# Bioinfo-Tools/PANGEA-plus

Measured on AMD Instinct MI355X. Metric: classified reads/sec (+ HBM GB/s fraction), 150 bp vs 1 Gbp db, 1/2/4/8 GPU, higher is better.
Workload: dtype u64 (2-bit packed bases, integer scores)

## Files before the change

pangea-plus_amd/csrc/classify.hip:

```cpp
#include <algorithm>
#include <chrono>

#include "bitops.hpp"
#include "consensus_core.hpp"
#include "engine.hpp"
#include "read_order.hpp"

#include <rocprim/device/device_radix_sort.hpp>

namespace pgx {

struct Diag {
	const uint64_t *rw, *ra;
	const uint64_t *dbw, *dba;
	int64_t dstart;
	int lo, hi;
};

template <bool AMB> __device__ __forceinline__ uint64_t mmw(const Diag &D, int w)
{
	int b0 = 32 * w;
	if (b0 + 32 <= D.lo || b0 >= D.hi)
		return kEven;
	uint64_t x = D.rw[w] ^ window64(D.dbw, D.dstart + b0);
// ... 1473 lines not shown
		const uint32_t k32 = kept ? dec_str_key32(rmv) : 0u;
		uint32_t kmax = k32;
#pragma unroll
		for (int m = 1; m < G; m <<= 1)
			kmax = max(kmax, (uint32_t)__shfl_xor(kmax, m));
		const bool elig = kept && k32 == kmax;
		if (PGX_SORT_DBG(cv) == 6) {
			if (__ballot(elig && slow && !present) && li == 0)
				recs[r].hit = 0;
			continue;
		}
		if (PGX_SORT_DBG(cv) != 4) {
			const uint32_t key2 = elig ? ((sim << 6) | (63u - rank)) + 1u : 0u;
			uint32_t top = key2;
#pragma unroll
			for (int m = 1; m < G; m <<= 1)
				top = max(top, (uint32_t)__shfl_xor(top, m));
			if (elig && key2 == top && present && !slow) {
				recs[r].hit = (int32_t)(o + rank);
				recs[r].matches = (int32_t)rmv;
			}
		}
		if (odd_mask) {
			const bool any_huge = __ballot(kept && (rmv >= 100000000u || ntok >= 100000000u || sim >= (1u << 25))) != 0ull;
			lds_fence();
			if (any_huge) {
				if (kept) {
					sw->b.rm[slot0 + rank] = rmv;
					sw->b.sim[slot0 + rank] = sim;
					sw->b.krm[slot0 + rank] = dec_str_key(rmv);
					sw->b.kcnt[slot0 + rank] = dec_str_key(ntok);
				}
				lds_fence();
				if (li == 0 && n && slow && present) {
					ArgmaxState am;
					am.cursim = r == 0 ? cv.simrank_undef : cv.simrank_zero;
					for (uint32_t k = 0; k < n; k++)
						am.step_keys((int32_t)(o + k), sw->b.rm[slot0 + k], sw->b.krm[slot0 + k], sw->b.kcnt[slot0 + k],
							     sw->b.sim[slot0 + k]);
					recs[r].hit = am.win;
					recs[r].matches = (int32_t)am.maxrm;
				}
			} else {
				const uint32_t c32 = dec_str_key32(ntok);
				if (kept) {
					sw->c.kcnt[slot0 + rank] = c32;
					sw->c.sim_e[slot0 + rank] = sim | (elig ? 0x80000000u : 0u);
					sw->c.krm[slot0 + rank] = k32;
					sw->c.rm[slot0 + rank] = rmv;
				}
				lds_fence();
				if (n && slow && present) {
					const bool top_is_max = (sw->c.sim_e[slot0] >> 31) != 0u;
					const uint32_t init_sim = r == 0 ? cv.simrank_undef : cv.simrank_zero;
					if (top_is_max) {
						uint32_t nx = kNoRead;
						for (uint32_t t = 0; t < n; t++) {
							const uint32_t a = sw->c.kcnt[slot0 + t], b2 = sw->c.sim_e[slot0 + t];
							const bool cand = kept && t > rank && (b2 >> 31) && (a > c32 || (b2 & 0x7FFFFFFFu) > sim);
							nx = (cand && nx == kNoRead) ? t : nx;
						}
						if (kept)
							sw->c.nxt[slot0 + rank] = nx;
						lds_fence();
						if (li == 0) {
							uint32_t w = kNoRead;
							if (sw->c.rm[slot0] > 0u) {
								w = 0;
							} else {
								for (uint32_t t = 0; t < n && w == kNoRead; t++)
									if (sw->c.kcnt[slot0 + t] > 1u  || (sw->c.sim_e[slot0 + t] & 0x7FFFFFFFu) > init_sim)
										w = t;
							}
							if (w != kNoRead) {
								for (uint32_t nxw = sw->c.nxt[slot0 + w]; nxw != kNoRead; nxw = sw->c.nxt[slot0 + w])
									w = nxw;
								recs[r].hit = (int32_t)(o + w);
								recs[r].matches = (int32_t)sw->c.rm[slot0 + w];
							} else {
								recs[r].hit = -1;
								recs[r].matches = 0;
							}
						}
					} else if (li == 0) {
						uint32_t kr = 1u , mrm = 0, kc = 1u, cs = init_sim;
						int32_t win = -1;
						for (uint32_t k = 0; k < n; k++) {
							const uint32_t vkrm = sw->c.krm[slot0 + k], vrm = sw->c.rm[slot0 + k], vkc = sw->c.kcnt[slot0 + k],
								       vs = sw->c.sim_e[slot0 + k] & 0x7FFFFFFFu;
							if (vkrm > kr) {
								kr = vkrm;
								mrm = vrm;
								win = (int32_t)(o + k);
								cs = vs;
							}
							if ((vkc > kc || cs < vs) && vrm == mrm) {
								kc = vkc;
								win = (int32_t)(o + k);
								cs = vs;
							}
						}
						recs[r].hit = win;
						recs[r].matches = (int32_t)mrm;
					}
				}
			}
		}
		lds_fence();
	}
	if (G != 64 && lane == 0 && chunk_used < 64u && chunk_used > 0)
		for (uint32_t k = chunk_used; k < 64u; k++)
			next_list[chunk_base + k] = kNoRead;
}

__global__ void k_consensus_serial(const pgx_hit *__restrict__ hits, const uint32_t *__restrict__ off,
				   const uint32_t *__restrict__ cnt, const uint32_t *__restrict__ list, uint32_t n_list,
				   ConsView cv, pgx_consensus_rec *__restrict__ recs)
{
	uint32_t t = blockIdx.x * blockDim.x + threadIdx.x;
	if (t >= n_list)
		return;
	const uint32_t r = list ? list[t] : t;
	const uint32_t o = off[r], n = cnt[r];
	pgx_consensus_rec rec;
	rec.hit = n ? -1 : -2;
	rec.matches = 0;
	if (cv.rdp_present && !cv.rdp_present[r])
		rec.hit = -2;
	if (rec.hit == -1) {
		const uint32_t r0 = cv.rdp_off[r], r1 = cv.rdp_off[r + 1];
		ArgmaxState am;
		am.cursim = r == 0 ? cv.simrank_undef : cv.simrank_zero;
		for (uint32_t k = 0; k < n; k++) {
			const pgx_hit h = hits[o + k];
			uint32_t c;
			const uint32_t rm = hit_rank_matches(cv, (uint32_t)h.subject, r0, r1, &c);
			am.step((int32_t)(o + k), rm, c, hit_simrank(cv, h));
		}
		rec.hit = am.win;
		rec.matches = (int32_t)am.maxrm;
	}
	recs[r] = rec;
}

__global__ void k_slice_offsets(const uint32_t *__restrict__ off, const uint32_t *__restrict__ cnt, uint32_t first, uint32_t n,
				 uint32_t *__restrict__ off_out, uint32_t *__restrict__ cnt_out)
{
	const uint32_t i = blockIdx.x * blockDim.x + threadIdx.x;
	if (i <= n)
		off_out[i] = off[first + i] - off[first];
	if (i < n)
		cnt_out[i] = cnt[first + i];
}

__global__ void k_slice_hits(const pgx_hit *__restrict__ in, uint64_t base, uint64_t n_slots, uint32_t first, pgx_hit *__restrict__ out)
{
	for (uint64_t i = (uint64_t)blockIdx.x * blockDim.x + threadIdx.x; i < n_slots; i += (uint64_t)gridDim.x * blockDim.x) {
		pgx_hit h = in[base + i];
		h.read -= (int32_t)first;
		out[i] = h;
	}
}

static thread_local pgx_stage_times t_times;

static DbView db_view(const pgx_db *db)
{
	DbView v;
	v.words = db->d_words.data();
	v.amb = db->has_amb ? db->d_amb.data() : nullptr;
	v.seq_off = db->d_seq_off.data();
	v.blk_subj = db->d_blk_subj.data();
	v.blk_info = db->d_blk_info.data();
	v.post_ctx = db->d_post_ctx.data();
	v.amb_blk = db->has_amb ? db->d_amb_blk.data() : nullptr;
	v.bucket_off = db->d_bucket_off.data();
	v.postings = db->d_postings.data();
	v.n_seq = (uint32_t)db->n_seq;
	v.n_bases = db->n_bases;
	v.bits = db->index_bits;
	v.gapped = db->ungapped ? 0 : 1;
	v.deep_from = kGapDeepFrom;
#ifdef PGX_STAGE_PROBES
	v.dbg_stop = getenv("PGX_SEED_STOP") ? atoi(getenv("PGX_SEED_STOP")) : 0;
#else
	v.dbg_stop = 0;
#endif
	return v;
}

static ReadsView reads_view(const pgx_reads *rd)
{
	ReadsView v;
	v.fwd = rd->d_fwd.data();
	v.rc = rd->d_rc.data();
	v.fwd_amb = rd->has_amb ? rd->d_fwd_amb.data() : nullptr;
	v.rc_amb = rd->has_amb ? rd->d_rc_amb.data() : nullptr;
	v.len = rd->d_len.data();
	v.woff = rd->d_woff.data();
	v.n = (uint32_t)rd->n;
	v.list = nullptr;
	v.ticket = nullptr;
	v.dustwin_f = rd->has_dust ? rd->dustb.win_f.data() : nullptr;
	v.dustwin_r = rd->has_dust ? rd->dustb.win_r.data() : nullptr;
	v.dust_any = rd->has_dust ? rd->dustb.any.data() : nullptr;
	return v;
}

static ConsView cons_view(const pgx_db *db, const pgx_rdp *rdp)
{
	ConsView cv;
	memset(&cv, 0, sizeof cv);
#ifdef PGX_STAGE_PROBES
	cv.dbg = getenv("PGX_SORT_STOP") ? atoi(getenv("PGX_SORT_STOP")) : 0;
#else
	cv.dbg = 0;
#endif
	if (db && db->bound) {
		cv.subj_tok_off = db->d_subj_tok_off.data();
		cv.subj_tok = db->d_subj_tok.data();
		cv.tok_rank = db->d_tok_rank.data();
		cv.subj_pairs = db->d_subj_pairs.data();
		cv.pair_words = db->pair_words;
		cv.simrank_lut = db->d_simrank_lut.data();
		cv.simrank_len = db->d_simrank_len.data();
		cv.simrank_undef = db->simrank_undef;
		cv.simrank_zero = db->simrank_zero;
	}
	cv.np_max = db ? db->max_pairs : 15;
	cv.nr_max = rdp ? rdp->max_trip : kRdpRegs;
	if (rdp) {
		cv.rdp_off = rdp->d_off.data();
		cv.rdp_name = rdp->d_name.data();
		cv.rdp_rank = rdp->d_rank.data();
		cv.rdp_present = rdp->d_present.data();
		cv.rdp_code = rdp->d_code.data();
	}
	return cv;
}

struct StageEvents {
	static constexpr int kN = 10;
	hipEvent_t e[kN] = {};
	bool ok = false;
	int init()
	{
		if (ok)
			return 0;
		for (auto &x : e)
			PGX_HIP(hipEventCreate(&x));
		ok = true;
		return 0;
	}
	void mark(int i, hipStream_t s) { (void)hipEventRecord(e[i], s); }
	float ms(int a, int b) const
	{
		float t = 0;
		(void)hipEventElapsedTime(&t, e[a], e[b]);
		return t;
	}
};

__global__ __launch_bounds__(256) void k_merge_pieces(const pgx_hit *__restrict__ scratch, const uint32_t *__restrict__ piece_start,
						      const uint32_t *__restrict__ piece_off, const uint32_t *__restrict__ parent,
						      const uint32_t *__restrict__ qoff, uint32_t n_pieces, pgx_hit *__restrict__ hits,
						      unsigned long long hits_cap, unsigned long long scratch_cap)
{
	const uint32_t waves = gridDim.x * (blockDim.x / 64), lane = threadIdx.x & 63;
	for (uint32_t s = blockIdx.x * (blockDim.x / 64) + (threadIdx.x >> 6); s < n_pieces; s += waves) {
		const uint32_t o = piece_off[s], cnt = piece_off[s + 1] - o;
		if (cnt == 0 || (unsigned long long)o + cnt > hits_cap)
			continue;
		const uint32_t st = piece_start[s];
		if (st != kFragmented && (unsigned long long)st + cnt > scratch_cap)
			continue;
		const pgx_hit *src = st == kFragmented ? hits + o : scratch + st;
		const int32_t read = (int32_t)parent[s], shift = (int32_t)qoff[s];
		for (uint32_t i = lane; i < cnt; i += 64) {
			pgx_hit h = src[i];
			h.read = read;
			h.qstart += shift;
			h.qend += shift;
			hits[o + i] = h;
		}
	}
}

__global__ void k_piece_ranges(const uint32_t *__restrict__ piece_first, const uint32_t *__restrict__ piece_off, uint32_t n_reads,
			       uint32_t *__restrict__ read_off, uint32_t *__restrict__ read_cnt, uint32_t *__restrict__ read_start)
{
	const uint32_t r = blockIdx.x * blockDim.x + threadIdx.x;
	if (r > n_reads)
		return;
	const uint32_t o = piece_off[piece_first[r]];
	read_off[r] = o;
	if (r < n_reads) {
		read_cnt[r] = piece_off[piece_first[r + 1]] - o;
		read_start[r] = kFragmented;
	}
}

struct Workspace {
	hipStream_t stream = nullptr;
	StageEvents ev;
	DevBuf<unsigned long long> counters;
	unsigned long long *h_counters = nullptr;
	DevBuf<pgx_hit> scratch, ovf;
	DevBuf<uint8_t> scratch_key, ovf_key;
	DevBuf<uint8_t> scratch_reg;
	DevBuf<uint32_t> partial, cursor, big_list, read_start, mid_list;
	DevBuf<uint32_t> piece_cnt, piece_off, parent_start;
	DevBuf<pgx_consensus_rec> recs;
	GappedWork gapped;
	DustBufs dust;
	DevBuf<uint32_t> order_key_in, order_val_in, order_key, order_list;
	DevBuf<uint8_t> order_tmp;
	DevBuf<uint32_t> order_ticket;
	uint64_t order_n = 0;
	pgx_hits hits;
	uint64_t hit_cap_hint = 0, ovf_cap_hint = 0;
	double table_per_read_hint = 0.0;
	pgx_stage_times times;
	int device = -1;
	~Workspace()
	{
		if (h_counters)
			(void)hipHostFree(h_counters);
		if (stream)
			(void)hipStreamDestroy(stream);
	}
};
constexpr int kNCounters = 12;

static int workspace_of(pgx_db *db, Workspace **out)
{
	if (!db->work) {
		auto w = std::make_shared<Workspace>();
		PGX_HIP(hipGetDevice(&w->device));
		PGX_HIP(hipStreamCreate(&w->stream));
		PGX_HIP(hipHostMalloc((void **)&w->h_counters, (kNCounters + 3) * sizeof(unsigned long long)));
		PGX_TRY(w->ev.init());
		PGX_TRY(w->counters.alloc(kNCounters, 0, 0, true));
		db->work = w;
	}
	*out = static_cast<Workspace *>(db->work.get());
	return 0;
}

int db_stream(pgx_db *db, hipStream_t *out)
{
	Workspace *ws = nullptr;
	PGX_TRY(workspace_of(db, &ws));
	*out = ws->stream;
	return 0;
}

constexpr uint64_t kOrderMinReads = 1u << 22;
constexpr uint64_t kOrderMinDbBytes = 32ull << 20;
static bool order_wanted(const pgx_db *db, uint64_t class_reads)
{
	if (db->read_order == 1)
		return class_reads > 0;
	if (db->read_order == 2)
		return false;
	return class_reads >= kOrderMinReads && (uint64_t)db->n_bases / 4 >= kOrderMinDbBytes;
}

static int order_reads(const pgx_db *db, const DbView &dv, const ReadsView &rv, const pgx_reads *sr, Workspace &ws,
		       std::vector<int64_t> &ordered)
{
	hipStream_t st = ws.stream;
	const std::vector<pgx_reads::SearchClass> &classes = sr->classes;
	ordered.assign(classes.size(), -1);
	const int shift = read_order_shift(dv.n_bases), key_bits = read_order_key_bits(dv.n_bases);
	const uint32_t last_bin = read_order_last_bin(dv.n_bases);
	uint64_t total = 0;
	size_t tmp_bytes = 0;
	for (size_t c = 0; c < classes.size(); c++)
		if (order_wanted(db, classes[c].count)) {
			ordered[c] = (int64_t)total;
			total += classes[c].count;
			size_t bytes = 0;
			PGX_HIP(rocprim::radix_sort_pairs(nullptr, bytes, (uint32_t *)nullptr, (uint32_t *)nullptr, (uint32_t *)nullptr, (uint32_t *)nullptr,
							  (size_t)classes[c].count, 0, key_bits, st));
			tmp_bytes = std::max(tmp_bytes, bytes);
		}
	ws.order_n = total;
	if (total == 0)
		return 0;
	PGX_TRY(ws.order_key_in.ensure(total));
	PGX_TRY(ws.order_val_in.ensure(total));
	PGX_TRY(ws.order_key.ensure(total));
	PGX_TRY(ws.order_list.ensure(total));
	PGX_TRY(ws.order_tmp.ensure(tmp_bytes ? tmp_bytes : 1));
	PGX_TRY(ws.order_ticket.ensure(classes.size()));
	for (size_t c = 0; c < classes.size(); c++) {
		if (ordered[c] < 0)
			continue;
		const uint64_t o = (uint64_t)ordered[c], cn = classes[c].count;
		ReadsView cvw = rv;
		cvw.n = (uint32_t)cn;
		cvw.list = classes[c].listed ? sr->d_class_list.data() + classes[c].off : nullptr;
		hipLaunchKernelGGL(k_read_order_keys, dim3((unsigned)((cn + 255) / 256)), dim3(256), 0, st, dv, cvw, shift, last_bin, (uint32_t)c,
				   ws.order_key_in.data() + o, ws.order_val_in.data() + o);
		PGX_HIP(hipGetLastError());
		size_t bytes = ws.order_tmp.n;
		PGX_HIP(rocprim::radix_sort_pairs(ws.order_tmp.data(), bytes, ws.order_key_in.data() + o, ws.order_key.data() + o,
						  ws.order_val_in.data() + o, ws.order_list.data() + o, (size_t)cn, 0, key_bits, st));
	}
	trace_point("order_reads");
	return 0;
}

int search_pipeline(pgx_db *db, pgx_reads *rd, const pgx_rdp *rdp, pgx_hits *out, pgx_consensus_rec *d_recs)
{
	PGX_TRY(require_device());
	if (rdp && !db->bound)
		return fail(PGX_E_ARG, "consensus needs pgx_db_bind_taxonomy() first");
	if (rdp && rdp->n != rd->n)
		return fail(PGX_E_ARG, "RDP stream holds %lld reads, batch holds %lld", (long long)rdp->n, (long long)rd->n);
	std::lock_guard<std::mutex> lock(db->search_mu);
	static const bool laps_on = getenv("PGX_CALL_LAPS") != nullptr;
	const auto lap_t0 = std::chrono::steady_clock::now();
	auto lap = [&](const char *what) {
		if (laps_on)
			fprintf(stderr, "[pgx lap] %8.2f ms  %s\n", std::chrono::duration<double, std::milli>(std::chrono::steady_clock::now() - lap_t0).count(), what);
	};
	trace_point("search_pipeline: entered");
	Workspace *wsp = nullptr;
	PGX_TRY(workspace_of(db, &wsp));
	Workspace &ws = *wsp;
	hipStream_t st = ws.stream;
	pgx_stage_times &tm = ws.times;
	memset(&tm, 0, sizeof tm);
	ws.order_n = 0;
	const uint64_t n = (uint64_t)rd->n;
	out->n_reads = rd->n;
	PGX_TRY(out->d_read_cnt.ensure(n + 1));
	PGX_TRY(out->d_read_off.ensure(n + 1));
	if (n == 0) {
		out->n_hits = 0;
		t_times = tm;
		return 0;
	}
	index_check(db, "search_pipeline");
	const DbView dv = db_view(db);
	const bool split = rd->pieces && rd->pieces->n > 0;
	const pgx_reads *sr = split ? rd->pieces.get() : rd;
	const uint64_t ns = (uint64_t)sr->n;
	if (split) {
		PGX_TRY(ws.piece_cnt.ensure(ns + 1));
		PGX_TRY(ws.piece_off.ensure(ns + 1));
		PGX_TRY(ws.parent_start.ensure(n));
	}
	ReadsView rv = reads_view(sr);
	if (!db->dust)
		rv.dustwin_f = rv.dustwin_r = nullptr;
	const int grid = (int)std::min<uint64_t>((n + kWavesPerBlock - 1) / kWavesPerBlock, 256ull * 8);

	uint64_t cap = std::max<uint64_t>(std::max<uint64_t>(std::max(n, ns) * 40, 1 << 16) + 256ull * 8 * kWavesPerBlock * kChunk, ws.hit_cap_hint);
	uint64_t ovf_cap = std::max<uint64_t>(std::max<uint64_t>(std::max(n, ns) / 4, 1 << 16), ws.ovf_cap_hint);
	uint64_t table_cap = std::max<uint64_t>(std::max<uint64_t>(std::max(n, ns) * 36, 1 << 16), (uint64_t)((double)std::max(n, ns) * ws.table_per_read_hint) + 1);
	DevBuf<pgx_hit> &scratch = ws.scratch, &ovf = ws.ovf;
	DevBuf<uint32_t> &read_start = ws.read_start;
	PGX_TRY(read_start.ensure(std::max(n, ns)));
	unsigned long long *h_cnt = ws.h_counters;
	const std::vector<pgx_reads::SearchClass> &classes = sr->classes;
	bool long_reads = false;
	for (auto &c : classes)
		long_reads = long_reads || c.words == 0;
	const uint32_t n_part = (uint32_t)((ns + kScanBlock * kScanItems - 1) / (kScanBlock * kScanItems));
	PGX_TRY(ws.partial.ensure(n_part));
	PGX_TRY(ws.cursor.ensure(ns));
	PGX_TRY(ws.big_list.ensure(n));
	PGX_TRY(ws.mid_list.ensure(n + 64ull * kWavesPerBlock * 256 * 8));
	trace_point("search_pipeline: lists ready");
	const ConsView cv = cons_view(db, rdp);
	const int lds_ok = rd->max_len <= 65535 ? 1 : 0;
	uint64_t H = 0, H_ovf = 0;
	ws.ev.mark(6, st);
	const bool dust_now = db->dust && db->dust_each_search;
	if (dust_now) {
		PGX_TRY(reads_dust_again(sr, ws.dust, st));
		if (sr->has_dust) {
			rv.dustwin_f = ws.dust.win_f.data();
			rv.dustwin_r = ws.dust.win_r.data();
			rv.dust_any = ws.dust.any.data();
		}
	}
	ws.ev.mark(7, st);
	std::vector<int64_t> ordered;
	PGX_TRY(order_reads(db, dv, rv, sr, ws, ordered));
	const bool order_now = ws.order_n > 0;
	if (order_now)
		ws.ev.mark(8, st);
	for (int attempt = 0;; attempt++) {
		if (attempt > 8)
			return fail(PGX_E_LIMIT, "hit tables did not settle after %d attempts", attempt);
		PGX_TRY(scratch.ensure(cap));
		PGX_TRY(ovf.ensure(ovf_cap));
		trace_point("search_pipeline: seed tables ready");
		PGX_TRY(out->d_hits.ensure(table_cap));
		trace_point("search_pipeline: hit table ready");
		cap = scratch.n;
		ovf_cap = ovf.n;
		if (dv.gapped) {
			PGX_TRY(ws.scratch_key.ensure(cap + 16));
			PGX_TRY(ws.scratch_reg.ensure(cap + 16));
			PGX_TRY(ws.ovf_key.ensure(ovf_cap));
			PGX_HIP(hipMemsetAsync(ws.scratch_key.data(), 0xFF, cap + 16, st));
		}
		table_cap = out->d_hits.n;
		PGX_HIP(hipMemsetAsync(ws.counters.data(), 0, kNCounters * sizeof(unsigned long long), st));
		OutView ov;
		ov.main = scratch.data();
		ov.ovf = ovf.data();
		ov.main_key = ws.scratch_key.data();
		ov.ovf_key = ws.ovf_key.data();
		ov.main_reg = ws.scratch_reg.data();
		ov.reg_shift = gapped_region_shift(db->n_bases);
		ov.main_cap = cap;
		ov.ovf_cap = ovf_cap;
		ov.counters = ws.counters.data();
		uint32_t *big_count = reinterpret_cast<uint32_t *>(ws.counters.data() + 8), *mid_count = reinterpret_cast<uint32_t *>(ws.counters.data() + 9);
		trace_point("search_pipeline: tables ready");
		lap("tables ready");
		if (order_now)
			PGX_HIP(hipMemsetAsync(ws.order_ticket.data(), 0, classes.size() * sizeof(uint32_t), st));
		ws.ev.mark(0, st);
		uint32_t *rc_ptr = split ? ws.piece_cnt.data() : out->d_read_cnt.data(), *rs_ptr = read_start.data();
		for (size_t ci = 0; ci < classes.size(); ci++) {
			pgx_reads::SearchClass c = classes[ci];
			c.amb = c.amb || db->has_amb;
			ReadsView cvw = rv;
			const uint64_t cn = c.count;
			cvw.n = (uint32_t)cn;
			cvw.list = c.listed ? sr->d_class_list.data() + c.off : nullptr;
			if (ordered[ci] >= 0) {
				c.listed = true;
				cvw.list = ws.order_list.data() + ordered[ci];
				cvw.ticket = ws.order_ticket.data() + ci;
			}
			const int per_block = kWavesPerBlock * (c.words > 0 ? 2 : 1);
			const dim3 g((unsigned)std::min<uint64_t>((cn + per_block - 1) / per_block, 256ull * 8)), b(64 * kWavesPerBlock);
#define PGX_SEED_LAUNCH2(A, W, D)                                                                                                  \
	do {                                                                                                                       \
		if (c.listed)                                                                                                      \
			hipLaunchKernelGGL((k_seed_extend<A, W, true, D>), g, b, 0, st, dv, cvw, ov, rc_ptr, rs_ptr);             \
		else                                                                                                               \
			hipLaunchKernelGGL((k_seed_extend<A, W, false, D>), g, b, 0, st, dv, cvw, ov, rc_ptr, rs_ptr);            \
	} while (0)
#define PGX_SEED_LAUNCH(A, W)                                                                                                      \
	do {                                                                                                                       \
		if (c.dust && cvw.dustwin_f)                                                                                       \
			PGX_SEED_LAUNCH2(A, W, true);                                                                              \
		else                                                                                                               \
			PGX_SEED_LAUNCH2(A, W, false);                                                                             \
	} while (0)
			if (c.amb && c.words == 3)
				PGX_SEED_LAUNCH(true, 3);
			else if (c.amb && c.words == 5)
				PGX_SEED_LAUNCH(true, 5);
			else if (c.amb && c.words == 8)
				PGX_SEED_LAUNCH(true, 8);
			else if (c.amb)
				PGX_SEED_LAUNCH(true, 0);
			else if (c.words == 3)
				PGX_SEED_LAUNCH(false, 3);
			else if (c.words == 5)
				PGX_SEED_LAUNCH(false, 5);
			else if (c.words == 8)
				PGX_SEED_LAUNCH(false, 8);
			else
				PGX_SEED_LAUNCH(false, 0);
#undef PGX_SEED_LAUNCH
#undef PGX_SEED_LAUNCH2
		}
		PGX_HIP(hipGetLastError());
		trace_point("k_seed_extend");
		ws.ev.mark(1, st);

		if (dv.gapped) {
			ReadsView all = rv;
			all.n = (uint32_t)ns;
			PGX_TRY(gapped_stage(dv, all, scratch.data(), ws.scratch_key.data(), rs_ptr, rc_ptr, ovf.data(), ws.ovf_key.data(),
					     ws.counters.data() + 4, ovf_cap, long_reads, cap, (int)sr->max_len, ws.gapped, st, ws.counters.data(), ws.scratch_reg.data()));
			trace_point("gapped_stage");
		}
		ws.ev.mark(2, st);

		const uint32_t *unit_cnt = split ? ws.piece_cnt.data() : out->d_read_cnt.data();
		uint32_t *unit_off = split ? ws.piece_off.data() : out->d_read_off.data();
		hipLaunchKernelGGL(k_scan_partials, dim3(n_part), dim3(kScanBlock), 0, st, unit_cnt, ns, ws.partial.data());
		hipLaunchKernelGGL(k_scan_top, dim3(1), dim3(kScanBlock), 0, st, ws.partial.data(), n_part);
		hipLaunchKernelGGL(k_scan_final, dim3(n_part), dim3(kScanBlock), 0, st, unit_cnt, ns, ws.partial.data(), unit_off);
		PGX_HIP(hipMemsetAsync(ws.cursor.data(), 0, ns * sizeof(uint32_t), st));
		hipLaunchKernelGGL(k_scatter_hits, dim3(256), dim3(256), 0, st, ovf.data(), ws.counters.data() + 4, ovf_cap, unit_off,
				   ws.cursor.data(), out->d_hits.data(), table_cap);
		PGX_HIP(hipGetLastError());
		const uint32_t *sort_start = read_start.data();
		if (split) {
			hipLaunchKernelGGL(k_merge_pieces, dim3((unsigned)std::min<uint64_t>((ns + 3) / 4, 256ull * 32)), dim3(256), 0, st, scratch.data(),
					   read_start.data(), ws.piece_off.data(), rd->d_piece_parent.data(), rd->d_piece_qoff.data(), (uint32_t)ns,
					   out->d_hits.data(), table_cap, cap);
			hipLaunchKernelGGL(k_piece_ranges, dim3((unsigned)((n + 1 + 255) / 256)), dim3(256), 0, st, rd->d_piece_first.data(),
					   ws.piece_off.data(), (uint32_t)n, out->d_read_off.data(), out->d_read_cnt.data(), ws.parent_start.data());
			PGX_HIP(hipGetLastError());
			sort_start = ws.parent_start.data();
		}
		trace_point("group");
		ws.ev.mark(3, st);

		const int grid2 = (int)std::min<uint64_t>((n + 2 * kWavesPerBlock - 1) / (2 * kWavesPerBlock), 256ull * 8);
		hipLaunchKernelGGL(k_sort_consensus<32>, dim3(grid2), dim3(64 * kWavesPerBlock), 0, st, out->d_hits.data(), scratch.data(),
				   sort_start, out->d_read_off.data(), out->d_read_cnt.data(), (unsigned long long)table_cap, (unsigned long long)cap, (uint32_t)n,
				   (const uint32_t *)nullptr, (const uint32_t *)nullptr, cv, rdp ? 1 : 0, lds_ok, d_recs, ws.mid_list.data(), mid_count);
		trace_point("k_sort_consensus<32>");
		hipLaunchKernelGGL(k_sort_consensus<64>, dim3(grid), dim3(64 * kWavesPerBlock), 0, st, out->d_hits.data(), scratch.data(),
				   sort_start, out->d_read_off.data(), out->d_read_cnt.data(), (unsigned long long)table_cap, (unsigned long long)cap, (uint32_t)n,
				   ws.mid_list.data(), mid_count, cv, rdp ? 1 : 0, lds_ok, d_recs, ws.big_list.data(), big_count);
		PGX_HIP(hipGetLastError());
		trace_point("k_sort_consensus<64>");
		ws.ev.mark(4, st);

		PGX_HIP(hipMemcpyAsync(h_cnt, ws.counters.data(), kNCounters * sizeof(unsigned long long), hipMemcpyDeviceToHost, st));
		h_cnt[kNCounters] = 0;
		h_cnt[kNCounters + 2] = 0;
		if (dv.gapped) {
			PGX_HIP(hipMemcpyAsync(h_cnt + kNCounters, ws.gapped.big_count.data(), 2 * sizeof(uint32_t), hipMemcpyDeviceToHost, st));
			PGX_HIP(hipMemcpyAsync(h_cnt + kNCounters + 2, ws.gapped.big_count.data() + 4, 2 * sizeof(uint32_t), hipMemcpyDeviceToHost, st));
		}
		PGX_HIP(hipMemcpyAsync(h_cnt + kNCounters + 1, out->d_read_off.data() + n, sizeof(uint32_t), hipMemcpyDeviceToHost, st));
		lap("step enqueued");
		PGX_HIP(hipStreamSynchronize(st));
		lap("step finished");
		H_ovf = h_cnt[4];
		H = h_cnt[5] + H_ovf;
		const uint64_t gap_listed = std::max<uint64_t>((uint32_t)h_cnt[kNCounters], (uint32_t)(h_cnt[kNCounters] >> 32)), gap_cap = ws.gapped.big_list.n;
		bool again = false;
		if (h_cnt[0] > cap) {
			cap = h_cnt[0] + h_cnt[0] / 8;
			again = true;
			tm.grown |= 1;
		}
		if (H_ovf > ovf_cap) {
			ovf_cap = H_ovf + H_ovf / 8;
			again = true;
			tm.grown |= 2;
		}
		if (dv.gapped && gap_listed > gap_cap) {
			PGX_TRY(ws.gapped.big_list.ensure(gap_listed + gap_listed / 8));
			again = true;
			tm.grown |= 4;
		}
		if (!again && H > table_cap) {
			table_cap = H + H / 16;
			again = true;
			tm.grown |= 8;
		}
		tm.attempts = attempt + 1;
		if (!again)
			break;
	}
	ws.hit_cap_hint = std::max<uint64_t>(ws.hit_cap_hint, h_cnt[0] + h_cnt[0] / 16);
	ws.ovf_cap_hint = std::max<uint64_t>(ws.ovf_cap_hint, H_ovf + H_ovf / 16);
	ws.table_per_read_hint = std::max(ws.table_per_read_hint, (double)(H + H / 16) / (double)std::max(n, ns));
	out->n_hits = (int64_t)H;
	out->gapped = dv.gapped != 0;
	tm.hits = (int64_t)H;
	tm.probes = (int64_t)h_cnt[1];
	tm.postings = (int64_t)h_cnt[2];
	tm.candidates = (int64_t)h_cnt[3];
	tm.survivors = (int64_t)h_cnt[6];
	tm.gapped_wide = (int64_t)(uint32_t)h_cnt[kNCounters] + (int64_t)(uint32_t)(h_cnt[kNCounters + 2] >> 32);
	tm.seed_extend_ms = ws.ev.ms(0, 1) + (order_now ? ws.ev.ms(7, 8) : 0.0f);
	tm.gapped_ms = ws.ev.ms(1, 2);
	tm.group_ms = ws.ev.ms(2, 3);
	tm.sort_ms = ws.ev.ms(3, 4);
	tm.total_ms = ws.ev.ms(0, 4) + (order_now ? ws.ev.ms(7, 8) : 0.0f);
	tm.dust_ms = dust_now ? ws.ev.ms(6, 7) : 0.0f;
	tm.total_ms += tm.dust_ms;
	const unsigned long long hit_limit = getenv("PGX_HIT_LIMIT") ? strtoull(getenv("PGX_HIT_LIMIT"), nullptr, 10) : (1ull << 32);
	if (H >= hit_limit)
		return fail(PGX_E_LIMIT, "%llu hits in one batch exceed the 32-bit slot limit: use smaller batches",
			    (unsigned long long)H);
	const uint32_t n_big = (uint32_t)h_cnt[8];
	if (n_big) {
		const uint32_t *sort_start = split ? ws.parent_start.data() : read_start.data();
		ws.ev.mark(4, st);
		PGX_TRY(sort_big_reads(out->d_hits.data(), scratch.data(), sort_start, out->d_read_off.data(), out->d_read_cnt.data(),
				       ws.big_list.data(), n_big, dv.gapped != 0));
		if (rdp) {
			hipLaunchKernelGGL(k_consensus_serial, dim3((n_big + 63) / 64), dim3(64), 0, 0, out->d_hits.data(), out->d_read_off.data(),
					   out->d_read_cnt.data(), ws.big_list.data(), n_big, cv, d_recs);
			PGX_HIP(hipGetLastError());
		}
		ws.ev.mark(5, 0);
		PGX_HIP(hipDeviceSynchronize());
		const float extra = ws.ev.ms(4, 5);
		tm.sort_ms += extra;
		tm.total_ms += extra;
	}
	t_times = tm;
	lap("done");
	trace_point("search_pipeline: done");
	return 0;
}

int consensus_device(const pgx_db *db, const pgx_hits *hits, const pgx_rdp *rdp, pgx_consensus_rec *d_out, pgx_stage_times *)
{
	if (!db->bound)
		return fail(PGX_E_ARG, "consensus needs pgx_db_bind_taxonomy() first");
	if (rdp->n != hits->n_reads)
		return fail(PGX_E_ARG, "RDP stream and hit table cover different read counts");
	const uint32_t n = (uint32_t)hits->n_reads;
	if (n == 0)
		return 0;
	const ConsView cv = cons_view(db, rdp);
	hipLaunchKernelGGL(k_consensus_serial, dim3((n + 63) / 64), dim3(64), 0, 0, hits->d_hits.data(), hits->d_read_off.data(),
			   hits->d_read_cnt.data(), (const uint32_t *)nullptr, n, cv, d_out);
	PGX_HIP(hipGetLastError());
	PGX_HIP(hipDeviceSynchronize());
	return 0;
}

}

using namespace pgx;

extern "C" {

int pgx_blast_search(pgx_db *db, pgx_reads *reads, pgx_hits **out)
{
	if (!db || !reads || !out)
		return fail(PGX_E_ARG, "pgx_blast_search: null argument");
	std::unique_ptr<pgx_hits> h(new pgx_hits());
	PGX_TRY(search_pipeline(db, reads, nullptr, h.get(), nullptr));
	*out = h.release();
	return 0;
}

int pgx_classify_consensus(pgx_db *db, pgx_reads *reads, const pgx_rdp *rdp, pgx_hits **hits_out, pgx_consensus_rec *out,
			   int64_t cap)
{
	if (!db || !reads || !rdp)
		return fail(PGX_E_ARG, "pgx_classify_consensus: null argument");
	Workspace *ws = nullptr;
	{
		std::lock_guard<std::mutex> lock(db->search_mu);
		PGX_TRY(workspace_of(db, &ws));
		PGX_TRY(ws->recs.ensure((size_t)reads->n + 1));
	}
	std::unique_ptr<pgx_hits> own(hits_out ? new pgx_hits() : nullptr);
	PGX_TRY(search_pipeline(db, reads, rdp, own ? own.get() : &ws->hits, ws->recs.data()));
	if (out) {
		if (cap < reads->n)
			return fail(PGX_E_ARG, "record buffer too small");
		PGX_TRY(ws->recs.download(out, (size_t)reads->n));
		trace_point("pgx_classify_consensus: records downloaded");
	}
	if (hits_out)
		*hits_out = own.release();
	return 0;
}

int pgx_classify_consensus_tri(pgx_db *db, pgx_reads *reads, const pgx_rdp *rdp, const char *soap_stream_path, pgx_hits **hits_out,
			       pgx_consensus_rec *out, int64_t cap)
{
	if (soap_stream_path && *soap_stream_path && strcmp(soap_stream_path, "0") != 0) {
		FILE *f = fopen(soap_stream_path, "r");
		if (!f)
			return fail(PGX_E_IO, "Error: Unable to open %s file.", soap_stream_path);
		fclose(f);
	}
	return pgx_classify_consensus(db, reads, rdp, hits_out, out, cap);
}

int pgx_db_get_dust(pgx_db *db, const pgx_reads *r, uint8_t *any_out, uint32_t *woff_out, uint64_t *mask_out, uint64_t *win_f_out,
		    uint64_t *win_r_out, int64_t cap_words, int64_t *n_words_out)
{
	if (!db || !r)
		return fail(PGX_E_ARG, "pgx_db_get_dust: null argument");
	if (r->pieces && r->pieces->n > 0)
		return fail(PGX_E_ARG, "pgx_db_get_dust: the batch is searched piece by piece, the handle's bits describe the pieces");
	std::lock_guard<std::mutex> lock(db->search_mu);
	if (!db->work)
		return fail(PGX_E_ARG, "pgx_db_get_dust: no search has run through this handle");
	const Workspace &ws = *static_cast<const Workspace *>(db->work.get());
	return dust_read_back("pgx_db_get_dust", r, ws.dust, ws.stream, any_out, woff_out, mask_out, win_f_out, win_r_out, cap_words, n_words_out);
}

int pgx_db_set_dust_each_search(pgx_db *db, int on)
{
	if (!db)
		return fail(PGX_E_ARG, "pgx_db_set_dust_each_search: null argument");
	db->dust_each_search = on != 0;
	return 0;
}

int pgx_db_set_read_order(pgx_db *db, int mode)
{
	if (!db || mode < 0 || mode > 2)
		return fail(PGX_E_ARG, "pgx_db_set_read_order: null handle, or a mode other than 0 (auto), 1 (always), 2 (never)");
	std::lock_guard<std::mutex> lock(db->search_mu);
	db->read_order = mode;
	return 0;
}

int pgx_db_get_read_order(pgx_db *db, const pgx_reads *r, uint32_t *order_out, uint32_t *key_out, int64_t cap, int64_t *n_out)
{
	if (!db || !r || !n_out)
		return fail(PGX_E_ARG, "pgx_db_get_read_order: null argument");
	std::lock_guard<std::mutex> lock(db->search_mu);
	if (!db->work)
		return fail(PGX_E_ARG, "pgx_db_get_read_order: no search has run through this handle");
	const Workspace &ws = *static_cast<const Workspace *>(db->work.get());
	const pgx_reads *sr = r->pieces && r->pieces->n > 0 ? r->pieces.get() : r;
	if ((int64_t)ws.order_n > sr->n)
		return fail(PGX_E_ARG, "pgx_db_get_read_order: the last search through this handle was given another batch");
	*n_out = (int64_t)ws.order_n;
	if (!order_out && !key_out)
		return 0;
	if (cap < (int64_t)ws.order_n)
		return fail(PGX_E_ARG, "pgx_db_get_read_order: room for %lld entries, the list holds %lld", (long long)cap, (long long)ws.order_n);
	PGX_HIP(hipStreamSynchronize(ws.stream));
	if (order_out)
		PGX_TRY(ws.order_list.download(order_out, (size_t)ws.order_n));
	if (key_out)
		PGX_TRY(ws.order_key.download(key_out, (size_t)ws.order_n));
	return 0;
}

int pgx_db_set_ungapped(pgx_db *db, int ungapped)
{
	if (!db)
		return fail(PGX_E_ARG, "pgx_db_set_ungapped: null argument");
	std::lock_guard<std::mutex> lock(db->search_mu);
	db->ungapped = ungapped != 0;
	return 0;
}

int pgx_db_set_dust(pgx_db *db, int dust)
{
	if (!db)
		return fail(PGX_E_ARG, "pgx_db_set_dust: null argument");
	std::lock_guard<std::mutex> lock(db->search_mu);
	db->dust = dust != 0;
	return 0;
}

void pgx_hits_close(pgx_hits *h) { delete h; }
int64_t pgx_hits_count(const pgx_hits *h) { return h ? h->n_hits : 0; }

int pgx_hits_copy(const pgx_hits *h, pgx_hit *out, int64_t cap)
{
	if (!h || !out || cap < h->n_hits)
		return fail(PGX_E_ARG, "pgx_hits_copy: bad argument");
	return h->d_hits.download(out, (size_t)h->n_hits);
}

int pgx_hits_slice(const pgx_hits *h, int64_t first_read, int64_t n_reads, pgx_hits **out)
{
	if (!h || !out || first_read < 0 || n_reads < 0 || first_read + n_reads > h->n_reads)
		return fail(PGX_E_ARG, "pgx_hits_slice: reads [%lld, +%lld) are not inside a table of %lld reads", (long long)first_read,
			    (long long)n_reads, (long long)(h ? h->n_reads : 0));
	PGX_TRY(require_device());
	return guard("pgx_hits_slice", [&]() -> int {
		std::unique_ptr<pgx_hits> s(new pgx_hits);
		s->n_reads = n_reads;
		s->gapped = h->gapped;
		PGX_TRY(s->d_read_off.alloc((size_t)n_reads + 1));
		PGX_TRY(s->d_read_cnt.alloc((size_t)n_reads + 1));
		uint32_t ends[2] = { 0, 0 };
		PGX_TRY(h->d_read_off.download(&ends[0], 1, (size_t)first_read));
		PGX_TRY(h->d_read_off.download(&ends[1], 1, (size_t)(first_read + n_reads)));
		const uint64_t n_slots = (uint64_t)ends[1] - ends[0];
		s->n_hits = (int64_t)n_slots;
		PGX_TRY(s->d_hits.alloc(n_slots ? n_slots : 1));
		hipLaunchKernelGGL(k_slice_offsets, dim3((unsigned)((n_reads + 1 + 255) / 256)), dim3(256), 0, 0, h->d_read_off.data(), h->d_read_cnt.data(),
				   (uint32_t)first_read, (uint32_t)n_reads, s->d_read_off.data(), s->d_read_cnt.data());
		if (n_slots)
			hipLaunchKernelGGL(k_slice_hits, dim3((unsigned)std::min<uint64_t>((n_slots + 255) / 256, 256ull * 32)), dim3(256), 0, 0, h->d_hits.data(),
					   (uint64_t)ends[0], n_slots, (uint32_t)first_read, s->d_hits.data());
		PGX_HIP(hipGetLastError());
		PGX_HIP(hipDeviceSynchronize());
		*out = s.release();
		return 0;
	});
}

int pgx_hits_read_offsets(const pgx_hits *h, int64_t *out, int64_t cap)
{
	if (!h || !out || cap < h->n_reads + 1)
		return fail(PGX_E_ARG, "pgx_hits_read_offsets: bad argument");
	std::vector<uint32_t> tmp((size_t)h->n_reads + 1);
	PGX_TRY(h->d_read_off.download(tmp.data(), tmp.size()));
	for (size_t i = 0; i < tmp.size(); i++)
		out[i] = tmp[i];
	return 0;
}

int pgx_hits_read_counts(const pgx_hits *h, int64_t *out, int64_t cap)
{
	if (!h || !out || cap < h->n_reads)
		return fail(PGX_E_ARG, "pgx_hits_read_counts: bad argument");
	std::vector<uint32_t> tmp((size_t)h->n_reads);
	PGX_TRY(h->d_read_cnt.download(tmp.data(), tmp.size()));
	for (size_t i = 0; i < tmp.size(); i++)
		out[i] = tmp[i];
	return 0;
}

int pgx_last_stage_times(pgx_stage_times *out)
{
	if (!out)
		return fail(PGX_E_ARG, "pgx_last_stage_times: null argument");
	*out = t_times;
	return 0;
}
}
```

Measured before the change: 128.0 million.

## Overlap read ordering and table fills with dust masking on a side stream

```diff
diff --git a/pangea-plus_amd/csrc/classify.hip b/pangea-plus_amd/csrc/classify.hip
--- a/pangea-plus_amd/csrc/classify.hip
+++ b/pangea-plus_amd/csrc/classify.hip
@@ -1799,6 +1799,8 @@
 
 struct Workspace {
 	hipStream_t stream = nullptr;
+	hipStream_t side = nullptr;
+	hipEvent_t fork = nullptr, join = nullptr;
 	StageEvents ev;
 	DevBuf<unsigned long long> counters;
 	unsigned long long *h_counters = nullptr;
@@ -1823,6 +1825,12 @@
 	{
 		if (h_counters)
 			(void)hipHostFree(h_counters);
+		if (fork)
+			(void)hipEventDestroy(fork);
+		if (join)
+			(void)hipEventDestroy(join);
+		if (side)
+			(void)hipStreamDestroy(side);
 		if (stream)
 			(void)hipStreamDestroy(stream);
 	}
@@ -1835,6 +1843,9 @@
 		auto w = std::make_shared<Workspace>();
 		PGX_HIP(hipGetDevice(&w->device));
 		PGX_HIP(hipStreamCreate(&w->stream));
+		PGX_HIP(hipStreamCreate(&w->side));
+		PGX_HIP(hipEventCreateWithFlags(&w->fork, hipEventDisableTiming));
+		PGX_HIP(hipEventCreateWithFlags(&w->join, hipEventDisableTiming));
 		PGX_HIP(hipHostMalloc((void **)&w->h_counters, (kNCounters + 3) * sizeof(unsigned long long)));
 		PGX_TRY(w->ev.init());
 		PGX_TRY(w->counters.alloc(kNCounters, 0, 0, true));
@@ -1863,10 +1874,9 @@
 	return class_reads >= kOrderMinReads && (uint64_t)db->n_bases / 4 >= kOrderMinDbBytes;
 }
 
-static int order_reads(const pgx_db *db, const DbView &dv, const ReadsView &rv, const pgx_reads *sr, Workspace &ws,
+static int order_reads(const pgx_db *db, const DbView &dv, const ReadsView &rv, const pgx_reads *sr, Workspace &ws, hipStream_t st,
 		       std::vector<int64_t> &ordered)
 {
-	hipStream_t st = ws.stream;
 	const std::vector<pgx_reads::SearchClass> &classes = sr->classes;
 	ordered.assign(classes.size(), -1);
 	const int shift = read_order_shift(dv.n_bases), key_bits = read_order_key_bits(dv.n_bases);
@@ -1975,25 +1985,7 @@
 	const ConsView cv = cons_view(db, rdp);
 	const int lds_ok = rd->max_len <= 65535 ? 1 : 0;
 	uint64_t H = 0, H_ovf = 0;
-	ws.ev.mark(6, st);
-	const bool dust_now = db->dust && db->dust_each_search;
-	if (dust_now) {
-		PGX_TRY(reads_dust_again(sr, ws.dust, st));
-		if (sr->has_dust) {
-			rv.dustwin_f = ws.dust.win_f.data();
-			rv.dustwin_r = ws.dust.win_r.data();
-			rv.dust_any = ws.dust.any.data();
-		}
-	}
-	ws.ev.mark(7, st);
-	std::vector<int64_t> ordered;
-	PGX_TRY(order_reads(db, dv, rv, sr, ws, ordered));
-	const bool order_now = ws.order_n > 0;
-	if (order_now)
-		ws.ev.mark(8, st);
-	for (int attempt = 0;; attempt++) {
-		if (attempt > 8)
-			return fail(PGX_E_LIMIT, "hit tables did not settle after %d attempts", attempt);
+	auto ensure_tables = [&]() -> int {
 		PGX_TRY(scratch.ensure(cap));
 		PGX_TRY(ovf.ensure(ovf_cap));
 		trace_point("search_pipeline: seed tables ready");
@@ -2001,14 +1993,55 @@
 		trace_point("search_pipeline: hit table ready");
 		cap = scratch.n;
 		ovf_cap = ovf.n;
+		table_cap = out->d_hits.n;
 		if (dv.gapped) {
 			PGX_TRY(ws.scratch_key.ensure(cap + 16));
 			PGX_TRY(ws.scratch_reg.ensure(cap + 16));
 			PGX_TRY(ws.ovf_key.ensure(ovf_cap));
-			PGX_HIP(hipMemsetAsync(ws.scratch_key.data(), 0xFF, cap + 16, st));
-		}
-		table_cap = out->d_hits.n;
-		PGX_HIP(hipMemsetAsync(ws.counters.data(), 0, kNCounters * sizeof(unsigned long long), st));
+		}
+		return 0;
+	};
+	auto fill_tables = [&](hipStream_t s) -> int {
+		if (dv.gapped)
+			PGX_HIP(hipMemsetAsync(ws.scratch_key.data(), 0xFF, cap + 16, s));
+		PGX_HIP(hipMemsetAsync(ws.counters.data(), 0, kNCounters * sizeof(unsigned long long), s));
+		return 0;
+	};
+	PGX_TRY(ensure_tables());
+	std::vector<int64_t> ordered;
+	const bool dust_now = db->dust && db->dust_each_search;
+	ws.ev.mark(6, st);
+	PGX_HIP(hipEventRecord(ws.fork, st));
+	const int prologue = [&]() -> int {
+		PGX_HIP(hipStreamWaitEvent(ws.side, ws.fork, 0));
+		PGX_TRY(order_reads(db, dv, rv, sr, ws, ws.side, ordered));
+		PGX_TRY(fill_tables(ws.side));
+		PGX_HIP(hipEventRecord(ws.join, ws.side));
+		if (dust_now) {
+			PGX_TRY(reads_dust_again(sr, ws.dust, st));
+			if (sr->has_dust) {
+				rv.dustwin_f = ws.dust.win_f.data();
+				rv.dustwin_r = ws.dust.win_r.data();
+				rv.dust_any = ws.dust.any.data();
+			}
+		}
+		ws.ev.mark(7, st);
+		PGX_HIP(hipStreamWaitEvent(st, ws.join, 0));
+		return 0;
+	}();
+	if (prologue != 0) {
+		(void)hipStreamSynchronize(ws.side);
+		return prologue;
+	}
+	ws.ev.mark(8, st);
+	const bool order_now = ws.order_n > 0;
+	for (int attempt = 0;; attempt++) {
+		if (attempt > 8)
+			return fail(PGX_E_LIMIT, "hit tables did not settle after %d attempts", attempt);
+		if (attempt > 0) {
+			PGX_TRY(ensure_tables());
+			PGX_TRY(fill_tables(st));
+		}
 		OutView ov;
 		ov.main = scratch.data();
 		ov.ovf = ovf.data();
@@ -2170,13 +2203,13 @@
 	tm.candidates = (int64_t)h_cnt[3];
 	tm.survivors = (int64_t)h_cnt[6];
 	tm.gapped_wide = (int64_t)(uint32_t)h_cnt[kNCounters] + (int64_t)(uint32_t)(h_cnt[kNCounters + 2] >> 32);
-	tm.seed_extend_ms = ws.ev.ms(0, 1) + (order_now ? ws.ev.ms(7, 8) : 0.0f);
+	const float exposed_ms = ws.ev.ms(7, 8);
+	tm.seed_extend_ms = ws.ev.ms(0, 1) + exposed_ms;
 	tm.gapped_ms = ws.ev.ms(1, 2);
 	tm.group_ms = ws.ev.ms(2, 3);
 	tm.sort_ms = ws.ev.ms(3, 4);
-	tm.total_ms = ws.ev.ms(0, 4) + (order_now ? ws.ev.ms(7, 8) : 0.0f);
 	tm.dust_ms = dust_now ? ws.ev.ms(6, 7) : 0.0f;
-	tm.total_ms += tm.dust_ms;
+	tm.total_ms = tm.dust_ms + exposed_ms + ws.ev.ms(0, 4);
 	const unsigned long long hit_limit = getenv("PGX_HIT_LIMIT") ? strtoull(getenv("PGX_HIT_LIMIT"), nullptr, 10) : (1ull << 32);
 	if (H >= hit_limit)
 		return fail(PGX_E_LIMIT, "%llu hits in one batch exceed the 32-bit slot limit: use smaller batches",
```

New measurement: 111.5 million. 0.871x the previous value.
